# DanielaCourel/smoothed_particle_hydrodynamics

Hardware: AMD Instinct MI355X
Metric: Mparticle-steps/sec (whole node), dam-break (higher is better)
Workload: dtype f32

## Files before the change

smoothed_particle_hydrodynamics_amd/csrc/cell_build.h:

```cpp
#pragma once

#include "sph_device.h"

#define SCAN_THREADS 256
#ifndef RANK_UNROLL
#define RANK_UNROLL 4
#endif
#ifndef RANK_BIG
#define RANK_BIG 512
#endif
#define RANK_CHUNK 4096
#define RANK_BIG_BLOCKS 64
#define SCAN_ITEMS 16
#define SCAN_TILE (SCAN_THREADS * SCAN_ITEMS)

__device__ __forceinline__ void count_cell_runs(uint32_t c, bool live, int i,
                                                uint32_t* __restrict__ cell_count,
                                                uint32_t* __restrict__ slot, uint32_t trash)
{
   live = live && c != trash;
   const int lane = threadIdx.x & (SPH_WAVE - 1);
   const uint32_t prev = __shfl_up(c, 1);
   const bool head = (lane == 0) || (prev != c);
   const unsigned long long heads = __ballot(head);
   const unsigned long long below = heads & ((lane == 63) ? ~0ull : ((1ull << (lane + 1)) - 1ull));
   const int head_lane = 63 - __clzll(below);
   const unsigned long long above = (head_lane == 63) ? 0ull : (heads >> (head_lane + 1));
   const int run_len = above ? (__ffsll((long long)above)) : (SPH_WAVE - head_lane);
   uint32_t base = 0;
   if (live && head) base = atomicAdd(&cell_count[c], (uint32_t)run_len);
   base = __shfl(base, head_lane);
   if (live) slot[i] = base + (uint32_t)(lane - head_lane);
}

template <bool WRITE_VOX, bool CHECK_DEAD>
__global__ void __launch_bounds__(256)
k_hash_count(const float4* __restrict__ posm, const float4* __restrict__ velp,
             int32_t* __restrict__ meta, CellGrid g, SlabZone zone, uint32_t* __restrict__ key,
             uint32_t* __restrict__ slot, uint32_t* __restrict__ cell_count,
             int32_t* __restrict__ vox)
{
   const int i = blockIdx.x * blockDim.x + threadIdx.x;
   const bool live = i < meta[META_N_IN];
   uint32_t c = 0xffffffffu;
   if (live) {
      const float4 p = posm[i];
      int cx, cy, cz;
// ... 27 lines not shown
   count_cell_runs(c, live, i, cell_count, slot, (uint32_t)g.ncells);
}

__device__ __forceinline__ uint32_t wave_inclusive_scan(uint32_t v, int lane)
{
#pragma unroll
   for (int d = 1; d < SPH_WAVE; d <<= 1) {
      uint32_t t = __shfl_up(v, d);
      if (lane >= d) v += t;
   }
   return v;
}

__device__ __forceinline__ uint32_t block_exclusive_scan(uint32_t v, uint32_t* total)
{
   __shared__ uint32_t wave_sums[SCAN_THREADS / SPH_WAVE];
   const int lane = threadIdx.x & (SPH_WAVE - 1);
   const int w = threadIdx.x / SPH_WAVE;
   const uint32_t inc = wave_inclusive_scan(v, lane);
   if (lane == SPH_WAVE - 1) wave_sums[w] = inc;
   __syncthreads();
   uint32_t carry = 0, tot = 0;
#pragma unroll
   for (int k = 0; k < SCAN_THREADS / SPH_WAVE; k++) {
      const uint32_t s = wave_sums[k];
      if (k < w) carry += s;
      tot += s;
   }
   __syncthreads();
   *total = tot;
   return carry + inc - v;
}

__global__ void __launch_bounds__(SCAN_THREADS)
k_scan_reduce(const uint32_t* __restrict__ count, int ncells, uint32_t* __restrict__ part)
{
   const int base = blockIdx.x * SCAN_TILE + threadIdx.x * SCAN_ITEMS;
   uint32_t s = 0;
   if (base + SCAN_ITEMS <= ncells) {
      const uint4* p = reinterpret_cast<const uint4*>(count + base);
#pragma unroll
      for (int k = 0; k < SCAN_ITEMS / 4; k++) {
         const uint4 v = p[k];
         s += v.x + v.y + v.z + v.w;
      }
   } else {
      for (int k = 0; k < SCAN_ITEMS; k++)
         if (base + k < ncells) s += count[base + k];
   }
   uint32_t total;
   block_exclusive_scan(s, &total);
   if (threadIdx.x == 0) part[blockIdx.x] = total;
}

__global__ void __launch_bounds__(SCAN_THREADS)
k_scan_final(uint32_t* __restrict__ count, int ncells, const uint32_t* __restrict__ part,
             uint32_t* __restrict__ cell_start, uint32_t* __restrict__ big_cells, uint32_t limit,
             int32_t* __restrict__ meta)
{
   if (blockIdx.x == 0 && threadIdx.x == 0) big_cells[0] = 0u;
   const int base = blockIdx.x * SCAN_TILE + threadIdx.x * SCAN_ITEMS;
   uint32_t v[SCAN_ITEMS];
   uint32_t s = 0;
   const bool empty_tile = part[blockIdx.x] == 0u;
   if (empty_tile) {
#pragma unroll
      for (int k = 0; k < SCAN_ITEMS; k++) v[k] = 0u;
   } else if (base + SCAN_ITEMS <= ncells) {
      const uint4* p = reinterpret_cast<const uint4*>(count + base);
#pragma unroll
      for (int k = 0; k < SCAN_ITEMS / 4; k++) {
         const uint4 q = p[k];
         v[4 * k + 0] = q.x;
         v[4 * k + 1] = q.y;
         v[4 * k + 2] = q.z;
         v[4 * k + 3] = q.w;
      }
   } else {
#pragma unroll
      for (int k = 0; k < SCAN_ITEMS; k++) v[k] = (base + k < ncells) ? count[base + k] : 0u;
   }
#pragma unroll
   for (int k = 0; k < SCAN_ITEMS; k++) s += v[k];
   uint32_t before = 0;
   for (int t = threadIdx.x; t < (int)blockIdx.x; t += SCAN_THREADS) before += part[t];
   uint32_t carry;
   block_exclusive_scan(before, &carry);
   uint32_t total;
   uint32_t run = carry + block_exclusive_scan(s, &total);
   if (base + SCAN_ITEMS <= ncells) {
      uint4* o = reinterpret_cast<uint4*>(cell_start + base);
      uint4* z = reinterpret_cast<uint4*>(count + base);
#pragma unroll
      for (int k = 0; k < SCAN_ITEMS / 4; k++) {
         uint4 q;
         q.x = min(run, limit); run += v[4 * k + 0];
         q.y = min(run, limit); run += v[4 * k + 1];
         q.z = min(run, limit); run += v[4 * k + 2];
         q.w = min(run, limit); run += v[4 * k + 3];
         o[k] = q;
         if ((v[4 * k + 0] | v[4 * k + 1] | v[4 * k + 2] | v[4 * k + 3]) != 0u) z[k] = make_uint4(0, 0, 0, 0);
      }
   } else {
      for (int k = 0; k < SCAN_ITEMS; k++) {
         if (base + k < ncells) {
            cell_start[base + k] = min(run, limit);
            if (v[k] != 0u) count[base + k] = 0;
            run += v[k];
         }
      }
   }
   if (base <= ncells - 1 && ncells - 1 < base + SCAN_ITEMS) {
      cell_start[ncells] = min(run, limit);
      if (run > limit) atomicOr(&meta[META_ERRORS], 4);
   }
}

__global__ void __launch_bounds__(256)
k_scatter(const uint32_t* __restrict__ key, const uint32_t* __restrict__ slot,
          const uint32_t* __restrict__ cell_start, int32_t* __restrict__ meta,
          uint32_t* __restrict__ perm, int cells_per_plane, int ncells, int own_lo, int own_hi,
          int sum_lo, int sum_hi, int bnd_lo, int bnd_hi, int32_t* __restrict__ tile_stats,
          int32_t* __restrict__ clear_a, int32_t* __restrict__ clear_b,
          uint32_t* __restrict__ big_cells, uint32_t limit)
{
   const int i = blockIdx.x * blockDim.x + threadIdx.x;
   if (tile_stats && i < TSTAT_COUNT && i != TSTAT_BLOCKS) tile_stats[i] = 0;
   const int n_in = meta[META_N_IN];
   if (i < n_in) {
      const uint32_t c = key[i];
      if (c != (uint32_t)ncells) {
         const uint32_t first = cell_start[c], sl = slot[i];
         if (first + sl < limit) perm[first + sl] = (uint32_t)i;
         if (sl == 0u && cell_start[c + 1] - first > (uint32_t)RANK_BIG)
            big_cells[1u + atomicAdd(&big_cells[0], 1u)] = c;
      }
   }
   if (i == 0) {
      meta[META_N_LIVE] = (int)cell_start[ncells];
      meta[META_OWN_BEGIN] = (int)cell_start[own_lo * cells_per_plane];
      meta[META_OWN_END] = (int)cell_start[own_hi * cells_per_plane];
      meta[META_SUM_BEGIN] = (int)cell_start[sum_lo * cells_per_plane];
      meta[META_SUM_END] = (int)cell_start[sum_hi * cells_per_plane];
      meta[META_BND_LO_END] = (int)cell_start[bnd_lo * cells_per_plane];
      meta[META_BND_HI_BEGIN] = (int)cell_start[bnd_hi * cells_per_plane];
      if (clear_a) *clear_a = 0;
      if (clear_b) *clear_b = 0;
      if (tile_stats)
         tile_stats[TSTAT_BLOCKS] =
            (meta[META_SUM_END] - meta[META_SUM_BEGIN] + TILE_THREADS - 1) / TILE_THREADS;
   }
}

__global__ void __launch_bounds__(256)
k_rank_order(const uint32_t* __restrict__ perm, const uint32_t* __restrict__ key,
             const uint32_t* __restrict__ cell_start, const int32_t* __restrict__ meta,
             uint32_t* __restrict__ order)
{
   const int p = blockIdx.x * blockDim.x + threadIdx.x;
   if (p >= meta[META_N_IN]) return;
   const uint32_t i = perm[p];
   const uint32_t c = key[i];
   const uint32_t s = cell_start[c], e = cell_start[c + 1];
   if (e - s > (uint32_t)RANK_BIG) return;
   uint32_t rank = 0;
   for (uint32_t q0 = s; q0 < e; q0 += 8) {
      uint32_t other[8];
#pragma unroll
      for (int u = 0; u < 8; u++) other[u] = perm[q0 + u < e ? q0 + u : e - 1];
#pragma unroll
      for (int u = 0; u < 8; u++) rank += (q0 + u < e && other[u] < i) ? 1u : 0u;
   }
   order[s + rank] = i;
}

__device__ __forceinline__ void
rank_gather(int p, int block_p0, uint32_t* __restrict__ lds_id, const uint32_t* __restrict__ perm,
            const uint32_t* __restrict__ key, const uint32_t* __restrict__ cell_start,
            const int32_t* __restrict__ meta, int trash, const float4* __restrict__ posm_in,
            const float4* __restrict__ velp_in, float4* __restrict__ posm_out,
            float4* __restrict__ velp_out, uint32_t* __restrict__ remap = nullptr)
{
   const int n_in = (int)cell_start[trash];
   bool active = p < n_in;
   uint32_t i = 0, c = 0, s = 0, e = 0, id = 0;
   float4 v = make_float4(0.f, 0.f, 0.f, 0.f);
   if (active) {
      i = perm[p];
      c = key[i];
      v = velp_in[i];
      id = __float_as_uint(v.w);
   }
   lds_id[threadIdx.x] = id;
   if (active) {
      if (c == (uint32_t)trash) {
         active = false;
      } else {
         s = cell_start[c];
         e = cell_start[c + 1];
         if (e - s > (uint32_t)RANK_BIG) active = false;
      }
   }
   __syncthreads();
   if (!active) return;
   const uint32_t b0 = (uint32_t)block_p0;
   const uint32_t b1 = min(b0 + blockDim.x, (uint32_t)n_in);
   const uint32_t in_lo = max(s, b0), in_hi = min(e, b1);
   uint32_t rank = 0, same = 0;
   for (uint32_t q0 = in_lo; q0 < in_hi; q0 += 4) {
      uint32_t other[4];
#pragma unroll
      for (int u = 0; u < 4; u++) other[u] = lds_id[(q0 + u < in_hi ? q0 + u : in_hi - 1) - b0];
#pragma unroll
      for (int u = 0; u < 4; u++) {
         rank += (q0 + u < in_hi && other[u] < id) ? 1u : 0u;
         same += (q0 + u < in_hi && other[u] == id) ? 1u : 0u;
      }
   }
#pragma unroll
   for (int side = 0; side < 2; side++) {
      const uint32_t lo = side == 0 ? s : in_hi, hi = side == 0 ? in_lo : e;
      for (uint32_t q0 = lo; q0 < hi; q0 += RANK_UNROLL) {
         uint32_t other[RANK_UNROLL];
#pragma unroll
         for (int u = 0; u < RANK_UNROLL; u++) other[u] = perm[q0 + u < hi ? q0 + u : hi - 1];
#pragma unroll
         for (int u = 0; u < RANK_UNROLL; u++) other[u] = __float_as_uint(velp_in[other[u]].w);
#pragma unroll
         for (int u = 0; u < RANK_UNROLL; u++) {
            rank += (q0 + u < hi && other[u] < id) ? 1u : 0u;
            same += (q0 + u < hi && other[u] == id) ? 1u : 0u;
         }
      }
   }
   if (same > 1u) atomicOr(const_cast<int32_t*>(&meta[META_ERRORS]), 16);
   posm_out[s + rank] = posm_in[i];
   velp_out[s + rank] = v;
   if (remap) remap[i] = s + rank;
}

__global__ void __launch_bounds__(256)
k_rank_gather(const uint32_t* __restrict__ perm, const uint32_t* __restrict__ key,
              const uint32_t* __restrict__ cell_start, const int32_t* __restrict__ meta, int trash,
              const float4* __restrict__ posm_in, const float4* __restrict__ velp_in,
              float4* __restrict__ posm_out, float4* __restrict__ velp_out,
              uint32_t* __restrict__ remap)
{
   __shared__ uint32_t lds_id[256];
   rank_gather(blockIdx.x * blockDim.x + threadIdx.x, blockIdx.x * blockDim.x, lds_id, perm, key,
               cell_start, meta, trash, posm_in, velp_in, posm_out, velp_out, remap);
}

template <bool FULL>
__global__ void __launch_bounds__(256)
k_rank_big(const uint32_t* __restrict__ big_cells, const uint32_t* __restrict__ perm,
           const uint32_t* __restrict__ cell_start, const float4* __restrict__ posm_in,
           const float4* __restrict__ velp_in, float4* __restrict__ posm_out,
           float4* __restrict__ velp_out, uint32_t* __restrict__ order,
           uint32_t* __restrict__ scratch_key, uint32_t* __restrict__ scratch_src,
           uint32_t* __restrict__ remap)
{
   __shared__ uint32_t skey[RANK_CHUNK], ssrc[RANK_CHUNK];
   const int tid = threadIdx.x;
   const uint32_t nbig = big_cells[0];
   for (uint32_t b = blockIdx.x; b < nbig; b += gridDim.x) {
      const uint32_t c = big_cells[1u + b];
      const uint32_t s = cell_start[c], m = cell_start[c + 1] - s;
      const uint32_t nchunks = (m + RANK_CHUNK - 1) / RANK_CHUNK;
      for (uint32_t ch = 0; ch < nchunks; ch++) {
         const uint32_t base = ch * RANK_CHUNK;
         const uint32_t len = min((uint32_t)RANK_CHUNK, m - base);
         uint32_t padded = 256;
         while (padded < len) padded <<= 1;
         for (uint32_t t = tid; t < padded; t += 256) {
            uint32_t key = 0xffffffffu, src = 0u;
            if (t < len) {
               src = perm[s + base + t];
               key = FULL ? __float_as_uint(velp_in[src].w) : src;
            }
            skey[t] = key;
            ssrc[t] = src;
         }
         __syncthreads();
         for (uint32_t k2 = 2; k2 <= padded; k2 <<= 1) {
            for (uint32_t j = k2 >> 1; j > 0; j >>= 1) {
               for (uint32_t t = tid; t < padded; t += 256) {
                  const uint32_t partner = t ^ j;
                  if (partner > t) {
                     const bool up = (t & k2) == 0;
                     const uint32_t a = skey[t], bb = skey[partner];
                     if ((a > bb) == up) {
                        skey[t] = bb;
                        skey[partner] = a;
                        const uint32_t sa = ssrc[t];
                        ssrc[t] = ssrc[partner];
                        ssrc[partner] = sa;
                     }
                  }
               }
               __syncthreads();
            }
         }
         for (uint32_t t = tid; t < len; t += 256) {
            if (nchunks == 1) {
               const uint32_t src = ssrc[t];
               if (FULL) {
                  posm_out[s + t] = posm_in[src];
                  velp_out[s + t] = velp_in[src];
                  if (remap) remap[src] = s + t;
               } else {
                  order[s + t] = src;
               }
            } else {
               scratch_key[s + base + t] = skey[t];
               scratch_src[s + base + t] = ssrc[t];
            }
         }
         __syncthreads();
      }
      if (nchunks > 1) {
         for (uint32_t idx = tid; idx < m; idx += 256) {
            const uint32_t key = scratch_key[s + idx], mine = idx / RANK_CHUNK;
            uint32_t rank = idx % RANK_CHUNK;
            for (uint32_t ch = 0; ch < nchunks; ch++) {
               if (ch == mine) continue;
               const uint32_t* keys = scratch_key + s + ch * RANK_CHUNK;
               uint32_t lo = 0, hi = min((uint32_t)RANK_CHUNK, m - ch * RANK_CHUNK);
               while (lo < hi) {
                  const uint32_t mid = (lo + hi) >> 1;
                  if (keys[mid] < key) lo = mid + 1;
                  else hi = mid;
               }
               rank += lo;
            }
            const uint32_t src = scratch_src[s + idx];
            if (FULL) {
               posm_out[s + rank] = posm_in[src];
               velp_out[s + rank] = velp_in[src];
               if (remap) remap[src] = s + rank;
            } else {
               order[s + rank] = src;
            }
         }
         __syncthreads();
      }
   }
}

__global__ void __launch_bounds__(256)
k_permute_sums(const uint32_t* __restrict__ remap, const uint32_t* __restrict__ key,
               const int32_t* __restrict__ meta, uint32_t trash, const float* __restrict__ rho,
               const float4* __restrict__ acc, const int32_t* __restrict__ ncount,
               float* __restrict__ rho_out, float4* __restrict__ acc_out,
               int32_t* __restrict__ ncount_out)
{
   const int i = blockIdx.x * blockDim.x + threadIdx.x;
   if (i >= meta[META_N_IN] || key[i] == trash) return;
   const uint32_t j = remap[i];
   rho_out[j] = rho[i];
   acc_out[j] = acc[i];
   ncount_out[j] = ncount[i];
}
```

smoothed_particle_hydrodynamics_amd/csrc/context.h:

```cpp
#pragma once

#include <stdlib.h>
#include <string.h>

#include <memory>
#include <new>
#include <utility>

#include "cell_build.h"
#include "common_kernels.h"
#include "full_kernels.h"
#include "full_tiled.h"
#include "ref_kernels.h"
#include "sample_kernels.h"
#include "slab_kernels.h"
#include "slab_rccl.h"

namespace {

std::string g_create_error;

inline int div_up(int a, int b) { return (a + b - 1) / b; }

bool getenv_flag(const char* name)
// ... 83 lines not shown
   int growths = 0;

   ~SlabComm()
   {
      const RcclApi* api = comm ? rccl_api(nullptr) : nullptr;
      if (api) (void)api->CommDestroy(comm);
   }
};
#define SLAB_GROW_EVERY 16

struct sph_hip_context {
   sph_hip_params prm;
   int mode = 0;
   int device = 0;
   int capacity = 0;
   int n = 0;
   int n_owned = 0;
   DevBuf<int32_t> meta;
   int plane_lo = 0, plane_hi = 0, halo = 0;
   hipStream_t stream = nullptr;
   Stream own_stream;
   Event ev[EV_RING][7];
   long long ev_steps = 0;
   std::string err;

   CellGrid grid;

   DevBuf<float4> posm[2];
   DevBuf<float4> velp[2];
   int cur = 0;

   DevBuf<uint32_t> key;
   DevBuf<uint32_t> slot;
   DevBuf<uint32_t> perm;
   DevBuf<uint32_t> order;
   DevBuf<uint32_t> cell_count;
   DevBuf<uint32_t> cell_start;
   DevBuf<uint32_t> scan_part;
   DevBuf<uint32_t> big_cells;
   int scan_tiles = 0;

   DevBuf<float> rho;
   DevBuf<float4> velB;
   DevBuf<float> auxc;
   DevBuf<float4> acc;
   DevBuf<int32_t> ncount;
   DevBuf<TileDesc> tile_desc;
   DevBuf<uint32_t> nlist;
   DevBuf<uint32_t> nlist_overflow;
   int fast = 0;
   struct {
      int valid = 0;
      int fast = 0;
      float rho0 = 0.0f, stiffness = 0.0f, kernel3 = 0.0f;
   } terms;
   int uniform_mass = 0;
   int use_tiled = 1;
   int prehashed = 0;
   int no_prehash = 0, no_fused_integrate = 0, no_fused_slab = 0;
   Stream chunk_stream;
   Event ev_chunk_fork, ev_chunk_join;
   int chunked_giveups = -1;
   int slab_fused = 0;
   void* slab_msgs[2] = {nullptr, nullptr};
   int slab_msg_capacity = 0;
   int had_exchange = 0;
   int may_hold_dead = 0;
// ... 238 lines not shown
```

smoothed_particle_hydrodynamics_amd/csrc/full_tiled.h:

```cpp
#pragma once

#include "launch_policy.h"
#include "common_kernels.h"
#include "full_kernels.h"
#include "slab_kernels.h"

#if defined(SPH_ABLATE) && !defined(SPH_DIAGNOSTIC_BUILD)
#error "SPH_ABLATE is for diagnostic builds only: add -DSPH_DIAGNOSTIC_BUILD (tools/build_variant.sh does)"
#endif

#ifdef SPH_TRIPCOUNT
#ifndef SPH_DIAGNOSTIC_BUILD
#error "SPH_TRIPCOUNT is for diagnostic builds only: add -DSPH_DIAGNOSTIC_BUILD"
#endif
enum {
   TRIP_D_WAVES = 0, TRIP_D_CHUNKS_W, TRIP_D_TEST8_W, TRIP_D_TEST8_L, TRIP_D_SLOTS_L, TRIP_D_POPS_W,
   TRIP_D_POPS_L, TRIP_D_POPLOOPS_W, TRIP_D_SUMTRIPS_W, TRIP_D_SUMSLOTS_W, TRIP_D_LISTED_L, TRIP_D_LANES_L,
   TRIP_A_WAVES = 16, TRIP_A_PTRIPS_W, TRIP_A_CNT_L, TRIP_A_VTRIPS_W, TRIP_A_NV_L, TRIP_A_LANES_L,
   TRIP_COUNT = 32
};
__device__ unsigned long long g_trip[TRIP_COUNT];
struct TripCounters {
   unsigned int v[16];
   __device__ TripCounters() { for (int i = 0; i < 16; i++) v[i] = 0; }
// ... 127 lines not shown
      return d.D[k];
   }
};

typedef float __attribute__((ext_vector_type(2))) f32x2;
typedef float __attribute__((ext_vector_type(4))) f32x4;

__device__ __forceinline__ f32x4 lds_read4(const float* base, int i)
{
   return *reinterpret_cast<const f32x4*>(__builtin_assume_aligned(base + i, 16));
}

static_assert(DENSITY_UNROLL == LIST_BLOCK_ENTRIES && ACCEL_UNROLL == LIST_BLOCK_ENTRIES, "a trip of the list-driven loops is one block of the lists");
static_assert(TILE_CAP_MAX + TILE_PAD <= (1 << ListEntry<false>::TBITS) &&
                 TILE_CAP_MAX_WIDE + TILE_PAD <= (1 << ListEntry<true>::TBITS),
              "tile index must fit the list entry");

struct TileDesc {
   int D[9];
   int B[9];
   int total;
   int pad;
};

struct TileLds {
   float* x;
   float* y;
   float* z;
};

extern __shared__ __attribute__((aligned(16))) float tile_lds_dynamic[];

__device__ __forceinline__ void
tile_desc(int tile, int ntiles, const uint32_t* __restrict__ perm, const uint32_t* __restrict__ key,
          const uint32_t* __restrict__ cell_start, const int32_t* __restrict__ meta, CellGrid g,
          TileDesc* __restrict__ desc, const TileCaps& caps, int32_t* __restrict__ stats,
          uint32_t* __restrict__ giveup_density, uint32_t* __restrict__ giveup_accel)
{
   const int begin = meta[META_SUM_BEGIN], end = meta[META_SUM_END];
   const int p0 = begin + tile * TILE_THREADS;
   int most = -1;
   if (tile < ntiles && p0 < end) {
      const int plast = min(p0 + TILE_THREADS - 1, end - 1);
      const int c_first = (int)key[perm[p0]];
      const int c_last = (int)key[perm[plast]];
      TileDesc d;
      int G[9], len[9];
#pragma unroll
      for (int k = 0; k < 9; k++) {
         const int off = ((k / 3 - 1) * g.ny + (k % 3 - 1)) * g.nx;
         int lo = c_first + off - 1, hi = c_last + off + 1;
         lo = lo < 0 ? 0 : lo;
         hi = hi > g.ncells - 1 ? g.ncells - 1 : hi;
         G[k] = 0;
         len[k] = 0;
         if (hi >= lo) {
            G[k] = (int)cell_start[lo];
            len[k] = (int)cell_start[hi + 1] - G[k];
         }
      }
      int run = 0, chain_end = -1, chain_d = 0;
#pragma unroll
      for (int k = 0; k < 9; k++) {
         d.B[k] = run;
         if (len[k] == 0) {
            d.D[k] = run - G[k];
         } else if (G[k] <= chain_end) {
            const int seg_end = G[k] + len[k];
            d.D[k] = chain_d;
            if (seg_end > chain_end) {
               run += seg_end - chain_end;
               chain_end = seg_end;
            }
         } else {
            d.D[k] = chain_d = run - G[k];
            run += len[k];
            chain_end = G[k] + len[k];
         }
      }
      d.total = run;
      d.pad = 0;
      desc[tile] = d;
      most = run;
   }
   const bool lead = (threadIdx.x & (SPH_WAVE - 1)) == 0;
#pragma unroll
   for (int c = 0; c < TILE_CANDS; c++) {
      const int over = __popcll(__ballot(c < caps.n_cand && most > caps.cand[c]));
      if (lead && over) atomicAdd(&stats[TSTAT_OVER + c], over);
   }
   int wave_most = most;
#pragma unroll
   for (int o = SPH_WAVE / 2; o > 0; o >>= 1) wave_most = max(wave_most, __shfl_xor(wave_most, o));
   if (lead && wave_most > stats[TSTAT_MAX]) atomicMax(&stats[TSTAT_MAX], wave_most);
   if (most > caps.cap_density) giveup_density[atomicAdd(&stats[TSTAT_GIVEUP_DENSITY], 1)] = (uint32_t)tile;
   if (most > caps.cap_density || most > caps.cap_accel)
      giveup_accel[atomicAdd(&stats[TSTAT_GIVEUP_ACCEL], 1)] = (uint32_t)tile;
}

__global__ void __launch_bounds__(256)
k_rank_gather_tile_desc(int desc_blocks, int ntiles, const uint32_t* __restrict__ perm,
                        const uint32_t* __restrict__ key, const uint32_t* __restrict__ cell_start,
                        const int32_t* __restrict__ meta, CellGrid g,
                        const float4* __restrict__ posm_in, const float4* __restrict__ velp_in,
                        float4* __restrict__ posm_out, float4* __restrict__ velp_out,
                        TileDesc* __restrict__ desc, TileCaps caps, int32_t* __restrict__ stats,
                        uint32_t* __restrict__ giveup_density, uint32_t* __restrict__ giveup_accel,
                        uint32_t* __restrict__ remap)
{
   if ((int)blockIdx.x < desc_blocks) {
      tile_desc(blockIdx.x * blockDim.x + threadIdx.x, ntiles, perm, key, cell_start, meta, g, desc,
                caps, stats, giveup_density, giveup_accel);
      return;
   }
   __shared__ uint32_t lds_id[256];
   rank_gather((blockIdx.x - desc_blocks) * blockDim.x + threadIdx.x,
               (blockIdx.x - desc_blocks) * blockDim.x, lds_id, perm, key, cell_start, meta,
               g.ncells, posm_in, velp_in, posm_out, velp_out, remap);
}

__device__ __forceinline__ void tile_desc_load(const TileDesc* __restrict__ desc, int wg, TileDesc& sd)
{
   const int tid = threadIdx.x;
   if (tid < (int)(sizeof(TileDesc) / sizeof(int)))
      reinterpret_cast<int*>(&sd)[tid] = reinterpret_cast<const int*>(&desc[wg])[tid];
   __syncthreads();
}

__device__ __forceinline__ int xcd_workgroup(int block, int nblocks)
{
   const int q = nblocks / 8, r = nblocks % 8, x = block % 8;
   return (x < r ? x * (q + 1) : r * (q + 1) + (x - r) * q) + block / 8;
}

__device__ __forceinline__ void tile_load(const float4* __restrict__ posm, const TileDesc& sd,
                                          const TileLds& L)
{
   const int tid = threadIdx.x;
   const int total = sd.total;
   int B[9], D[9];
#pragma unroll
   for (int k = 0; k < 9; k++) {
      B[k] = sd.B[k];
      D[k] = sd.D[k];
   }
#if defined(SPH_ABLATE) && (SPH_ABLATE == 3 || SPH_ABLATE == 5)
   for (int base = 0; base < 0; base += TILE_BATCH * TILE_THREADS) {
#else
   for (int base = 0; base < total; base += TILE_BATCH * TILE_THREADS) {
#endif
      float4 buf[TILE_BATCH];
// ... 1070 lines not shown
```

smoothed_particle_hydrodynamics_amd/csrc/launch.h:

```cpp
#pragma once

#include <math.h>

#include <type_traits>

#include "context.h"

namespace {

template <class F>
void bind_flags(F&& f) { f(); }
template <class F, class... Rest>
void bind_flags(F&& f, bool flag, Rest... rest)
{
   if (flag) bind_flags([&](auto... later) { f(std::true_type{}, later...); }, rest...);
   else bind_flags([&](auto... later) { f(std::false_type{}, later...); }, rest...);
}

PairConsts pair_consts(const sph_hip_params& p, bool fast)
{
   PairConsts k;
   k.h2 = p.h2;
   static const float screen = getenv("SPH_HIP_TEST_SCREEN") ? (float)atof(getenv("SPH_HIP_TEST_SCREEN"))
                                                             : TEST_SCREEN_FACTOR;
// ... 172 lines not shown
   const SlabZone zone = slab_zone(ctx);
   if (ctx->prehashed == 2) {
      ctx->prehashed = 0;
      hipLaunchKernelGGL(k_hash_tail, dim3(SLAB_PACK_BLOCKS), dim3(256), 0, st, ctx->posm[cur], ctx->meta, g,
                         ctx->key, ctx->slot, ctx->cell_count);
   } else if (ctx->prehashed) {
      ctx->prehashed = 0;
   } else {
      const bool ref = ctx->mode == SPH_HIP_MODE_REF;
      bind_flags([&](auto R, auto D) {
         if constexpr (!(R.value && D.value))
            hipLaunchKernelGGL((k_hash_count<R.value, D.value>), dim3(blocks), dim3(256), 0, st, ctx->posm[cur],
                               ctx->velp[cur], ctx->meta, g, zone, ctx->key, ctx->slot, ctx->cell_count,
                               R.value ? ctx->vox.get() : nullptr);
      }, ref, !ref && ctx->may_hold_dead != 0);
   }
   ctx->early_exchange = 0;
   ctx->may_hold_dead = 0;
   const int tiles = ctx->scan_tiles;
   const int ncells_scan = g.ncells + 1;
   hipLaunchKernelGGL(k_scan_reduce, dim3(tiles), dim3(SCAN_THREADS), 0, st, ctx->cell_count,
                      ncells_scan, ctx->scan_part);
   hipLaunchKernelGGL(k_scan_final, dim3(tiles), dim3(SCAN_THREADS), 0, st, ctx->cell_count,
                      ncells_scan, ctx->scan_part, ctx->cell_start, ctx->big_cells, (uint32_t)ctx->capacity,
                      ctx->meta);
   const PlaneRanges r = plane_ranges(ctx->plane_lo, ctx->plane_hi, g.z0, g.nz, ctx->halo, zone.have_left,
                                      zone.have_right);
   hipLaunchKernelGGL(k_scatter, dim3(blocks), dim3(256), 0, st, ctx->key, ctx->slot,
                      ctx->cell_start, ctx->meta, ctx->perm, g.nx * g.ny, g.ncells, r.own_lo, r.own_hi,
                      r.sum_lo, r.sum_hi, r.bnd_lo, r.bnd_hi, ctx->tile_stats, (int32_t*)clear_left,
                      (int32_t*)clear_right, ctx->big_cells, (uint32_t)ctx->capacity);
   uint32_t* scratch_key = reinterpret_cast<uint32_t*>(ctx->stage.get());
   uint32_t* scratch_src = scratch_key + ctx->capacity;
   uint32_t* remap = (keep_sums && ctx->mode == SPH_HIP_MODE_FULL && !ctx->had_exchange) ? ctx->slot : nullptr;
   if (ctx->mode == SPH_HIP_MODE_REF) {
      hipLaunchKernelGGL(k_rank_order, dim3(blocks), dim3(256), 0, st, ctx->perm, ctx->key,
                         ctx->cell_start, ctx->meta, ctx->order);
      hipLaunchKernelGGL(k_rank_big<false>, dim3(RANK_BIG_BLOCKS), dim3(256), 0, st, ctx->big_cells,
                         ctx->perm, ctx->cell_start, (const float4*)nullptr, (const float4*)nullptr,
                         (float4*)nullptr, (float4*)nullptr, ctx->order, scratch_key, scratch_src,
                         (uint32_t*)nullptr);
   } else {
      const int nxt = cur ^ 1;
      if (ctx->use_tiled) {
         static_assert(sizeof(TileDesc) == 20 * sizeof(int), "TileDesc is 20 ints");
         pick_tile_caps(ctx);
         const int ntiles = div_up(n, TILE_THREADS), desc_blocks = div_up(ntiles, 256);
         hipLaunchKernelGGL(k_rank_gather_tile_desc, dim3(desc_blocks + blocks), dim3(256), 0, st,
                            desc_blocks, ntiles, ctx->perm, ctx->key, ctx->cell_start, ctx->meta,
                            g, ctx->posm[cur], ctx->velp[cur], ctx->posm[nxt], ctx->velp[nxt],
                            ctx->tile_desc, ctx->caps, ctx->tile_stats, ctx->giveup_density,
                            ctx->giveup_accel, remap);
      } else {
         hipLaunchKernelGGL(k_rank_gather, dim3(blocks), dim3(256), 0, st, ctx->perm, ctx->key,
                            ctx->cell_start, ctx->meta, g.ncells, ctx->posm[cur], ctx->velp[cur],
                            ctx->posm[nxt], ctx->velp[nxt], remap);
      }
      hipLaunchKernelGGL(k_rank_big<true>, dim3(RANK_BIG_BLOCKS), dim3(256), 0, st, ctx->big_cells,
                         ctx->perm, ctx->cell_start, ctx->posm[cur], ctx->velp[cur], ctx->posm[nxt],
                         ctx->velp[nxt], (uint32_t*)nullptr, scratch_key, scratch_src, remap);
      if (remap) {
         ctx->terms.valid = 0;
         float4* acc_t = reinterpret_cast<float4*>(ctx->stage.get() + ((2 * (size_t)ctx->capacity + 3) & ~(size_t)3));
         float* rho_t = reinterpret_cast<float*>(acc_t + (size_t)ctx->capacity);
         int32_t* cnt_t = reinterpret_cast<int32_t*>(rho_t + (size_t)ctx->capacity);
         hipLaunchKernelGGL(k_permute_sums, dim3(blocks), dim3(256), 0, st, remap, ctx->key, ctx->meta,
                            (uint32_t)g.ncells, ctx->rho, ctx->acc, ctx->ncount, rho_t, acc_t, cnt_t);
         SPH_TRY(hipMemcpyAsync(ctx->rho, rho_t, sizeof(float) * n, hipMemcpyDeviceToDevice, st));
         SPH_TRY(hipMemcpyAsync(ctx->acc, acc_t, sizeof(float4) * n, hipMemcpyDeviceToDevice, st));
         SPH_TRY(hipMemcpyAsync(ctx->ncount, cnt_t, sizeof(int32_t) * n, hipMemcpyDeviceToDevice, st));
      }
      ctx->cur = nxt;
   }
   SPH_TRY(hipGetLastError());
   return SPH_HIP_OK;
}

int launch_find_neighbors(sph_hip_context* ctx)
{
   if (ctx->mode != SPH_HIP_MODE_REF || ctx->n == 0) return SPH_HIP_OK;
   const sph_hip_params& p = ctx->prm;
   hipLaunchKernelGGL(k_ref_find_neighbors, dim3(div_up(ctx->n, 256)), dim3(256), 0, ctx->stream,
                      ctx->posm[0], ctx->vox, ctx->cell_start, ctx->order, ctx->n, p.cells_x,
                      p.cells_y, p.cells_z, p.h, p.htimes2, p.h2, p.sim_scale, p.examine_count,
                      ctx->nb, ctx->nd, ctx->ncount);
   SPH_TRY(hipGetLastError());
   return SPH_HIP_OK;
}

struct SlabFused {
   void* left;
   void* right;
   int capacity;
// ... 291 lines not shown
```

Measured before the change: 4796.

## Pack cell id into perm, fuse big-cell ranking into gather kernel, restructure scan

The permutation array now stores the particle index and its cell id as a pair, so the rank, gather and tile-descriptor code no longer chase key[perm[p]]. The big-cell sort runs as extra leading blocks of the gather kernel (using a smaller LDS chunk) instead of a separate launch. Rank-gather finds cell bounds within its block from LDS run heads, which avoids most cell_start loads. The cell scan processes twice as many cells per tile with a wave-strided, coalesced uint4 layout. In exchange, perm traffic doubles, and the big-cell blocks now share LDS sizing and scheduling with the normal gather blocks.

```diff
diff --git a/smoothed_particle_hydrodynamics_amd/csrc/cell_build.h b/smoothed_particle_hydrodynamics_amd/csrc/cell_build.h
--- a/smoothed_particle_hydrodynamics_amd/csrc/cell_build.h
+++ b/smoothed_particle_hydrodynamics_amd/csrc/cell_build.h
@@ -11,8 +11,12 @@
 #endif
 #define RANK_CHUNK 4096
 #define RANK_BIG_BLOCKS 64
-#define SCAN_ITEMS 16
+#ifndef SCAN_ITEMS
+#define SCAN_ITEMS 32
+#endif
 #define SCAN_TILE (SCAN_THREADS * SCAN_ITEMS)
+#define SCAN_WAVE_CELLS (SCAN_TILE / (SCAN_THREADS / SPH_WAVE))
+#define SCAN_ROUNDS (SCAN_WAVE_CELLS / (4 * SPH_WAVE))
 
 __device__ __forceinline__ void count_cell_runs(uint32_t c, bool live, int i,
                                                 uint32_t* __restrict__ cell_count,
@@ -106,22 +110,32 @@
    return carry + inc - v;
 }
 
+__device__ __forceinline__ int scan_cell0(int tile)
+{
+   return tile * SCAN_TILE + (threadIdx.x / SPH_WAVE) * SCAN_WAVE_CELLS + 4 * (threadIdx.x & (SPH_WAVE - 1));
+}
+
+__device__ __forceinline__ uint4 scan_load4(const uint32_t* __restrict__ count, int c0, int ncells)
+{
+   if (c0 + 4 <= ncells) return *reinterpret_cast<const uint4*>(count + c0);
+   uint4 q;
+   q.x = c0 + 0 < ncells ? count[c0 + 0] : 0u;
+   q.y = c0 + 1 < ncells ? count[c0 + 1] : 0u;
+   q.z = c0 + 2 < ncells ? count[c0 + 2] : 0u;
+   q.w = c0 + 3 < ncells ? count[c0 + 3] : 0u;
+   return q;
+}
+
 __global__ void __launch_bounds__(SCAN_THREADS)
 k_scan_reduce(const uint32_t* __restrict__ count, int ncells, uint32_t* __restrict__ part)
 {
-   const int base = blockIdx.x * SCAN_TILE + threadIdx.x * SCAN_ITEMS;
+   const int cell0 = scan_cell0(blockIdx.x);
+   uint4 q[SCAN_ROUNDS];
+#pragma unroll
+   for (int r = 0; r < SCAN_ROUNDS; r++) q[r] = scan_load4(count, cell0 + r * 4 * SPH_WAVE, ncells);
    uint32_t s = 0;
-   if (base + SCAN_ITEMS <= ncells) {
-      const uint4* p = reinterpret_cast<const uint4*>(count + base);
-#pragma unroll
-      for (int k = 0; k < SCAN_ITEMS / 4; k++) {
-         const uint4 v = p[k];
-         s += v.x + v.y + v.z + v.w;
-      }
-   } else {
-      for (int k = 0; k < SCAN_ITEMS; k++)
-         if (base + k < ncells) s += count[base + k];
-   }
+#pragma unroll
+   for (int r = 0; r < SCAN_ROUNDS; r++) s += q[r].x + q[r].y + q[r].z + q[r].w;
    uint32_t total;
    block_exclusive_scan(s, &total);
    if (threadIdx.x == 0) part[blockIdx.x] = total;
@@ -133,67 +147,61 @@
              int32_t* __restrict__ meta)
 {
    if (blockIdx.x == 0 && threadIdx.x == 0) big_cells[0] = 0u;
-   const int base = blockIdx.x * SCAN_TILE + threadIdx.x * SCAN_ITEMS;
-   uint32_t v[SCAN_ITEMS];
-   uint32_t s = 0;
+   const int lane = threadIdx.x & (SPH_WAVE - 1);
+   const int cell0 = scan_cell0(blockIdx.x);
    const bool empty_tile = part[blockIdx.x] == 0u;
-   if (empty_tile) {
-#pragma unroll
-      for (int k = 0; k < SCAN_ITEMS; k++) v[k] = 0u;
-   } else if (base + SCAN_ITEMS <= ncells) {
-      const uint4* p = reinterpret_cast<const uint4*>(count + base);
-#pragma unroll
-      for (int k = 0; k < SCAN_ITEMS / 4; k++) {
-         const uint4 q = p[k];
-         v[4 * k + 0] = q.x;
-         v[4 * k + 1] = q.y;
-         v[4 * k + 2] = q.z;
-         v[4 * k + 3] = q.w;
-      }
-   } else {
-#pragma unroll
-      for (int k = 0; k < SCAN_ITEMS; k++) v[k] = (base + k < ncells) ? count[base + k] : 0u;
-   }
-#pragma unroll
-   for (int k = 0; k < SCAN_ITEMS; k++) s += v[k];
+   uint4 q[SCAN_ROUNDS];
+#pragma unroll
+   for (int r = 0; r < SCAN_ROUNDS; r++)
+      q[r] = empty_tile ? make_uint4(0, 0, 0, 0) : scan_load4(count, cell0 + r * 4 * SPH_WAVE, ncells);
    uint32_t before = 0;
    for (int t = threadIdx.x; t < (int)blockIdx.x; t += SCAN_THREADS) before += part[t];
    uint32_t carry;
    block_exclusive_scan(before, &carry);
+   uint32_t pre[SCAN_ROUNDS];
+   uint32_t wave_run = 0;
+#pragma unroll
+   for (int r = 0; r < SCAN_ROUNDS; r++) {
+      const uint32_t sum = q[r].x + q[r].y + q[r].z + q[r].w;
+      const uint32_t inc = wave_inclusive_scan(sum, lane);
+      pre[r] = wave_run + inc - sum;
+      wave_run += __shfl(inc, SPH_WAVE - 1);
+   }
    uint32_t total;
-   uint32_t run = carry + block_exclusive_scan(s, &total);
-   if (base + SCAN_ITEMS <= ncells) {
-      uint4* o = reinterpret_cast<uint4*>(cell_start + base);
-      uint4* z = reinterpret_cast<uint4*>(count + base);
-#pragma unroll
-      for (int k = 0; k < SCAN_ITEMS / 4; k++) {
-         uint4 q;
-         q.x = min(run, limit); run += v[4 * k + 0];
-         q.y = min(run, limit); run += v[4 * k + 1];
-         q.z = min(run, limit); run += v[4 * k + 2];
-         q.w = min(run, limit); run += v[4 * k + 3];
-         o[k] = q;
-         if ((v[4 * k + 0] | v[4 * k + 1] | v[4 * k + 2] | v[4 * k + 3]) != 0u) z[k] = make_uint4(0, 0, 0, 0);
-      }
-   } else {
-      for (int k = 0; k < SCAN_ITEMS; k++) {
-         if (base + k < ncells) {
-            cell_start[base + k] = min(run, limit);
-            if (v[k] != 0u) count[base + k] = 0;
-            run += v[k];
-         }
-      }
-   }
-   if (base <= ncells - 1 && ncells - 1 < base + SCAN_ITEMS) {
-      cell_start[ncells] = min(run, limit);
-      if (run > limit) atomicOr(&meta[META_ERRORS], 4);
+   const uint32_t run = carry + __shfl(block_exclusive_scan(lane == 0 ? wave_run : 0u, &total), 0);
+#pragma unroll
+   for (int r = 0; r < SCAN_ROUNDS; r++) {
+      const int c0 = cell0 + r * 4 * SPH_WAVE;
+      const uint32_t v[4] = {q[r].x, q[r].y, q[r].z, q[r].w};
+      uint32_t at = run + pre[r];
+      if (c0 + 4 <= ncells) {
+         uint4 o;
+         o.x = min(at, limit); at += v[0];
+         o.y = min(at, limit); at += v[1];
+         o.z = min(at, limit); at += v[2];
+         o.w = min(at, limit); at += v[3];
+         *reinterpret_cast<uint4*>(cell_start + c0) = o;
+         if ((v[0] | v[1] | v[2] | v[3]) != 0u) *reinterpret_cast<uint4*>(count + c0) = make_uint4(0, 0, 0, 0);
+      } else {
+         for (int k = 0; k < 4; k++) {
+            if (c0 + k < ncells) {
+               cell_start[c0 + k] = min(at, limit);
+               if (v[k] != 0u) count[c0 + k] = 0;
+               at += v[k];
+            }
+         }
+      }
+      if (c0 <= ncells - 1 && ncells - 1 < c0 + 4) {
+         cell_start[ncells] = min(at, limit);
+         if (at > limit) atomicOr(&meta[META_ERRORS], 4);
+      }
    }
 }
 
 __global__ void __launch_bounds__(256)
 k_scatter(const uint32_t* __restrict__ key, const uint32_t* __restrict__ slot,
           const uint32_t* __restrict__ cell_start, int32_t* __restrict__ meta,
-          uint32_t* __restrict__ perm, int cells_per_plane, int ncells, int own_lo, int own_hi,
+          uint2* __restrict__ perm, int cells_per_plane, int ncells, int own_lo, int own_hi,
           int sum_lo, int sum_hi, int bnd_lo, int bnd_hi, int32_t* __restrict__ tile_stats,
           int32_t* __restrict__ clear_a, int32_t* __restrict__ clear_b,
           uint32_t* __restrict__ big_cells, uint32_t limit)
@@ -205,7 +213,7 @@
       const uint32_t c = key[i];
       if (c != (uint32_t)ncells) {
          const uint32_t first = cell_start[c], sl = slot[i];
-         if (first + sl < limit) perm[first + sl] = (uint32_t)i;
+         if (first + sl < limit) perm[first + sl] = make_uint2((uint32_t)i, c);
          if (sl == 0u && cell_start[c + 1] - first > (uint32_t)RANK_BIG)
             big_cells[1u + atomicAdd(&big_cells[0], 1u)] = c;
       }
@@ -227,59 +235,76 @@
 }
 
 __global__ void __launch_bounds__(256)
-k_rank_order(const uint32_t* __restrict__ perm, const uint32_t* __restrict__ key,
-             const uint32_t* __restrict__ cell_start, const int32_t* __restrict__ meta,
+k_rank_order(const uint2* __restrict__ perm, const uint32_t* __restrict__ cell_start, int trash,
              uint32_t* __restrict__ order)
 {
    const int p = blockIdx.x * blockDim.x + threadIdx.x;
-   if (p >= meta[META_N_IN]) return;
-   const uint32_t i = perm[p];
-   const uint32_t c = key[i];
+   if (p >= (int)cell_start[trash]) return;
+   const uint2 pc = perm[p];
+   const uint32_t i = pc.x, c = pc.y;
    const uint32_t s = cell_start[c], e = cell_start[c + 1];
    if (e - s > (uint32_t)RANK_BIG) return;
    uint32_t rank = 0;
    for (uint32_t q0 = s; q0 < e; q0 += 8) {
       uint32_t other[8];
 #pragma unroll
-      for (int u = 0; u < 8; u++) other[u] = perm[q0 + u < e ? q0 + u : e - 1];
+      for (int u = 0; u < 8; u++) other[u] = perm[q0 + u < e ? q0 + u : e - 1].x;
 #pragma unroll
       for (int u = 0; u < 8; u++) rank += (q0 + u < e && other[u] < i) ? 1u : 0u;
    }
    order[s + rank] = i;
 }
 
+#define RANK_GATHER_WAVES (256 / SPH_WAVE)
+#define RANK_GATHER_LDS (2 * 256 + 2 * RANK_GATHER_WAVES)
 __device__ __forceinline__ void
-rank_gather(int p, int block_p0, uint32_t* __restrict__ lds_id, const uint32_t* __restrict__ perm,
-            const uint32_t* __restrict__ key, const uint32_t* __restrict__ cell_start,
-            const int32_t* __restrict__ meta, int trash, const float4* __restrict__ posm_in,
-            const float4* __restrict__ velp_in, float4* __restrict__ posm_out,
-            float4* __restrict__ velp_out, uint32_t* __restrict__ remap = nullptr)
-{
+rank_gather(int p, int block_p0, uint32_t* __restrict__ lds, const uint2* __restrict__ perm,
+            const uint32_t* __restrict__ cell_start, const int32_t* __restrict__ meta, int trash,
+            const float4* __restrict__ posm_in, const float4* __restrict__ velp_in,
+            float4* __restrict__ posm_out, float4* __restrict__ velp_out,
+            uint32_t* __restrict__ remap = nullptr)
+{
+   uint32_t* lds_c = lds;
+   uint32_t* lds_id = lds + 256;
+   int* wave_first = reinterpret_cast<int*>(lds + 512);
+   int* wave_last = wave_first + RANK_GATHER_WAVES;
+   const int tid = threadIdx.x, lane = tid & (SPH_WAVE - 1), w = tid / SPH_WAVE;
    const int n_in = (int)cell_start[trash];
    bool active = p < n_in;
-   uint32_t i = 0, c = 0, s = 0, e = 0, id = 0;
-   float4 v = make_float4(0.f, 0.f, 0.f, 0.f);
+   uint32_t i = 0, c = 0xffffffffu, id = 0;
+   float4 v = make_float4(0.f, 0.f, 0.f, 0.f), x = v;
    if (active) {
-      i = perm[p];
-      c = key[i];
+      const uint2 pc = perm[p];
+      i = pc.x;
+      c = pc.y;
       v = velp_in[i];
+      x = posm_in[i];
       id = __float_as_uint(v.w);
    }
-   lds_id[threadIdx.x] = id;
-   if (active) {
-      if (c == (uint32_t)trash) {
-         active = false;
-      } else {
-         s = cell_start[c];
-         e = cell_start[c + 1];
-         if (e - s > (uint32_t)RANK_BIG) active = false;
-      }
-   }
+   lds_c[tid] = c;
+   lds_id[tid] = id;
    __syncthreads();
-   if (!active) return;
+   const unsigned long long heads = __ballot(active && (tid == 0 || lds_c[tid - 1] != c));
+   if (lane == 0) {
+      wave_first[w] = heads ? w * SPH_WAVE + __ffsll((long long)heads) - 1 : 256;
+      wave_last[w] = heads ? w * SPH_WAVE + 63 - __clzll(heads) : -1;
+   }
+   __syncthreads();
+   if (!active || c == (uint32_t)trash) return;
+   const int nb = min(256, n_in - block_p0);
+   const unsigned long long below = heads & ((lane == 63) ? ~0ull : ((1ull << (lane + 1)) - 1ull));
+   int lo_l = below ? w * SPH_WAVE + 63 - __clzll(below) : 0;
+   if (!below)
+      for (int k = 0; k < w; k++) lo_l = max(lo_l, wave_last[k]);
+   const unsigned long long above = (lane == 63) ? 0ull : (heads >> (lane + 1));
+   int hi_l = above ? tid + __ffsll((long long)above) : nb;
+   if (!above)
+      for (int k = w + 1; k < RANK_GATHER_WAVES; k++) hi_l = min(hi_l, wave_first[k]);
    const uint32_t b0 = (uint32_t)block_p0;
-   const uint32_t b1 = min(b0 + blockDim.x, (uint32_t)n_in);
-   const uint32_t in_lo = max(s, b0), in_hi = min(e, b1);
+   const uint32_t in_lo = b0 + (uint32_t)lo_l, in_hi = b0 + (uint32_t)hi_l;
+   const uint32_t s = lo_l == 0 ? cell_start[c] : in_lo;
+   const uint32_t e = hi_l == nb ? cell_start[c + 1] : in_hi;
+   if (e - s > (uint32_t)RANK_BIG) return;
    uint32_t rank = 0, same = 0;
    for (uint32_t q0 = in_lo; q0 < in_hi; q0 += 4) {
       uint32_t other[4];
@@ -297,7 +322,7 @@
       for (uint32_t q0 = lo; q0 < hi; q0 += RANK_UNROLL) {
          uint32_t other[RANK_UNROLL];
 #pragma unroll
-         for (int u = 0; u < RANK_UNROLL; u++) other[u] = perm[q0 + u < hi ? q0 + u : hi - 1];
+         for (int u = 0; u < RANK_UNROLL; u++) other[u] = perm[q0 + u < hi ? q0 + u : hi - 1].x;
 #pragma unroll
          for (int u = 0; u < RANK_UNROLL; u++) other[u] = __float_as_uint(velp_in[other[u]].w);
 #pragma unroll
@@ -308,48 +333,36 @@
       }
    }
    if (same > 1u) atomicOr(const_cast<int32_t*>(&meta[META_ERRORS]), 16);
-   posm_out[s + rank] = posm_in[i];
+   posm_out[s + rank] = x;
    velp_out[s + rank] = v;
    if (remap) remap[i] = s + rank;
 }
 
-__global__ void __launch_bounds__(256)
-k_rank_gather(const uint32_t* __restrict__ perm, const uint32_t* __restrict__ key,
-              const uint32_t* __restrict__ cell_start, const int32_t* __restrict__ meta, int trash,
-              const float4* __restrict__ posm_in, const float4* __restrict__ velp_in,
-              float4* __restrict__ posm_out, float4* __restrict__ velp_out,
-              uint32_t* __restrict__ remap)
-{
-   __shared__ uint32_t lds_id[256];
-   rank_gather(blockIdx.x * blockDim.x + threadIdx.x, blockIdx.x * blockDim.x, lds_id, perm, key,
-               cell_start, meta, trash, posm_in, velp_in, posm_out, velp_out, remap);
-}
-
-template <bool FULL>
-__global__ void __launch_bounds__(256)
-k_rank_big(const uint32_t* __restrict__ big_cells, const uint32_t* __restrict__ perm,
-           const uint32_t* __restrict__ cell_start, const float4* __restrict__ posm_in,
-           const float4* __restrict__ velp_in, float4* __restrict__ posm_out,
-           float4* __restrict__ velp_out, uint32_t* __restrict__ order,
-           uint32_t* __restrict__ scratch_key, uint32_t* __restrict__ scratch_src,
-           uint32_t* __restrict__ remap)
-{
-   __shared__ uint32_t skey[RANK_CHUNK], ssrc[RANK_CHUNK];
+template <bool FULL, int CHUNK>
+__device__ void
+rank_big_cells(int block, int nblocks, uint32_t* __restrict__ skey, uint32_t* __restrict__ ssrc,
+               const uint32_t* __restrict__ big_cells, const uint2* __restrict__ perm,
+               const uint32_t* __restrict__ cell_start, const float4* __restrict__ posm_in,
+               const float4* __restrict__ velp_in, float4* __restrict__ posm_out,
+               float4* __restrict__ velp_out, uint32_t* __restrict__ order,
+               uint32_t* __restrict__ scratch_key, uint32_t* __restrict__ scratch_src,
+               uint32_t* __restrict__ remap)
+{
    const int tid = threadIdx.x;
    const uint32_t nbig = big_cells[0];
-   for (uint32_t b = blockIdx.x; b < nbig; b += gridDim.x) {
+   for (uint32_t b = block; b < nbig; b += nblocks) {
       const uint32_t c = big_cells[1u + b];
       const uint32_t s = cell_start[c], m = cell_start[c + 1] - s;
-      const uint32_t nchunks = (m + RANK_CHUNK - 1) / RANK_CHUNK;
+      const uint32_t nchunks = (m + CHUNK - 1) / CHUNK;
       for (uint32_t ch = 0; ch < nchunks; ch++) {
-         const uint32_t base = ch * RANK_CHUNK;
-         const uint32_t len = min((uint32_t)RANK_CHUNK, m - base);
+         const uint32_t base = ch * CHUNK;
+         const uint32_t len = min((uint32_t)CHUNK, m - base);
          uint32_t padded = 256;
          while (padded < len) padded <<= 1;
          for (uint32_t t = tid; t < padded; t += 256) {
             uint32_t key = 0xffffffffu, src = 0u;
             if (t < len) {
-               src = perm[s + base + t];
+               src = perm[s + base + t].x;
                key = FULL ? __float_as_uint(velp_in[src].w) : src;
             }
             skey[t] = key;
@@ -394,12 +407,12 @@
       }
       if (nchunks > 1) {
          for (uint32_t idx = tid; idx < m; idx += 256) {
-            const uint32_t key = scratch_key[s + idx], mine = idx / RANK_CHUNK;
-            uint32_t rank = idx % RANK_CHUNK;
+            const uint32_t key = scratch_key[s + idx], mine = idx / CHUNK;
+            uint32_t rank = idx % CHUNK;
             for (uint32_t ch = 0; ch < nchunks; ch++) {
                if (ch == mine) continue;
-               const uint32_t* keys = scratch_key + s + ch * RANK_CHUNK;
-               uint32_t lo = 0, hi = min((uint32_t)RANK_CHUNK, m - ch * RANK_CHUNK);
+               const uint32_t* keys = scratch_key + s + ch * CHUNK;
+               uint32_t lo = 0, hi = min((uint32_t)CHUNK, m - ch * CHUNK);
                while (lo < hi) {
                   const uint32_t mid = (lo + hi) >> 1;
                   if (keys[mid] < key) lo = mid + 1;
@@ -422,6 +435,56 @@
 }
 
 __global__ void __launch_bounds__(256)
+k_rank_big(const uint32_t* __restrict__ big_cells, const uint2* __restrict__ perm,
+           const uint32_t* __restrict__ cell_start, uint32_t* __restrict__ order,
+           uint32_t* __restrict__ scratch_key, uint32_t* __restrict__ scratch_src)
+{
+   __shared__ uint32_t skey[RANK_CHUNK], ssrc[RANK_CHUNK];
+   rank_big_cells<false, RANK_CHUNK>(blockIdx.x, gridDim.x, skey, ssrc, big_cells, perm, cell_start,
+                                     nullptr, nullptr, nullptr, nullptr, order, scratch_key, scratch_src,
+                                     nullptr);
+}
+
+#define RANK_CHUNK_GATHER 2048
+#define RANK_GATHER_SHARED (2 * RANK_CHUNK_GATHER)
+static_assert(RANK_GATHER_SHARED >= RANK_GATHER_LDS, "the big-cell sort's LDS holds the gather's");
+
+struct BigCellWork {
+   const uint32_t* big_cells;
+   uint32_t* scratch_key;
+   uint32_t* scratch_src;
+};
+
+__device__ __forceinline__ void
+gather_big_cells(int block, uint32_t* __restrict__ lds, const BigCellWork& big,
+                 const uint2* __restrict__ perm, const uint32_t* __restrict__ cell_start,
+                 const float4* __restrict__ posm_in, const float4* __restrict__ velp_in,
+                 float4* __restrict__ posm_out, float4* __restrict__ velp_out,
+                 uint32_t* __restrict__ remap)
+{
+   rank_big_cells<true, RANK_CHUNK_GATHER>(block, RANK_BIG_BLOCKS, lds, lds + RANK_CHUNK_GATHER,
+                                           big.big_cells, perm, cell_start, posm_in, velp_in, posm_out,
+                                           velp_out, nullptr, big.scratch_key, big.scratch_src, remap);
+}
+
+__global__ void __launch_bounds__(256)
+k_rank_gather(BigCellWork big, const uint2* __restrict__ perm,
+              const uint32_t* __restrict__ cell_start, const int32_t* __restrict__ meta, int trash,
+              const float4* __restrict__ posm_in, const float4* __restrict__ velp_in,
+              float4* __restrict__ posm_out, float4* __restrict__ velp_out,
+              uint32_t* __restrict__ remap)
+{
+   __shared__ uint32_t lds[RANK_GATHER_SHARED];
+   if ((int)blockIdx.x < RANK_BIG_BLOCKS) {
+      gather_big_cells(blockIdx.x, lds, big, perm, cell_start, posm_in, velp_in, posm_out, velp_out, remap);
+      return;
+   }
+   const int b = blockIdx.x - RANK_BIG_BLOCKS;
+   rank_gather(b * blockDim.x + threadIdx.x, b * blockDim.x, lds, perm, cell_start, meta, trash, posm_in,
+               velp_in, posm_out, velp_out, remap);
+}
+
+__global__ void __launch_bounds__(256)
 k_permute_sums(const uint32_t* __restrict__ remap, const uint32_t* __restrict__ key,
                const int32_t* __restrict__ meta, uint32_t trash, const float* __restrict__ rho,
                const float4* __restrict__ acc, const int32_t* __restrict__ ncount,
diff --git a/smoothed_particle_hydrodynamics_amd/csrc/context.h b/smoothed_particle_hydrodynamics_amd/csrc/context.h
--- a/smoothed_particle_hydrodynamics_amd/csrc/context.h
+++ b/smoothed_particle_hydrodynamics_amd/csrc/context.h
@@ -139,7 +139,7 @@
 
    DevBuf<uint32_t> key;
    DevBuf<uint32_t> slot;
-   DevBuf<uint32_t> perm;
+   DevBuf<uint2> perm;
    DevBuf<uint32_t> order;
    DevBuf<uint32_t> cell_count;
    DevBuf<uint32_t> cell_start;
diff --git a/smoothed_particle_hydrodynamics_amd/csrc/full_tiled.h b/smoothed_particle_hydrodynamics_amd/csrc/full_tiled.h
--- a/smoothed_particle_hydrodynamics_amd/csrc/full_tiled.h
+++ b/smoothed_particle_hydrodynamics_amd/csrc/full_tiled.h
@@ -183,7 +183,7 @@
 extern __shared__ __attribute__((aligned(16))) float tile_lds_dynamic[];
 
 __device__ __forceinline__ void
-tile_desc(int tile, int ntiles, const uint32_t* __restrict__ perm, const uint32_t* __restrict__ key,
+tile_desc(int tile, int ntiles, const uint2* __restrict__ perm,
           const uint32_t* __restrict__ cell_start, const int32_t* __restrict__ meta, CellGrid g,
           TileDesc* __restrict__ desc, const TileCaps& caps, int32_t* __restrict__ stats,
           uint32_t* __restrict__ giveup_density, uint32_t* __restrict__ giveup_accel)
@@ -193,8 +193,8 @@
    int most = -1;
    if (tile < ntiles && p0 < end) {
       const int plast = min(p0 + TILE_THREADS - 1, end - 1);
-      const int c_first = (int)key[perm[p0]];
-      const int c_last = (int)key[perm[plast]];
+      const int c_first = (int)perm[p0].y;
+      const int c_last = (int)perm[plast].y;
       TileDesc d;
       int G[9], len[9];
 #pragma unroll
@@ -250,8 +250,8 @@
 }
 
 __global__ void __launch_bounds__(256)
-k_rank_gather_tile_desc(int desc_blocks, int ntiles, const uint32_t* __restrict__ perm,
-                        const uint32_t* __restrict__ key, const uint32_t* __restrict__ cell_start,
+k_rank_gather_tile_desc(BigCellWork big, int desc_blocks, int ntiles, const uint2* __restrict__ perm,
+                        const uint32_t* __restrict__ cell_start,
                         const int32_t* __restrict__ meta, CellGrid g,
                         const float4* __restrict__ posm_in, const float4* __restrict__ velp_in,
                         float4* __restrict__ posm_out, float4* __restrict__ velp_out,
@@ -259,15 +259,21 @@
                         uint32_t* __restrict__ giveup_density, uint32_t* __restrict__ giveup_accel,
                         uint32_t* __restrict__ remap)
 {
-   if ((int)blockIdx.x < desc_blocks) {
-      tile_desc(blockIdx.x * blockDim.x + threadIdx.x, ntiles, perm, key, cell_start, meta, g, desc,
-                caps, stats, giveup_density, giveup_accel);
+   __shared__ uint32_t lds[RANK_GATHER_SHARED];
+   int b = blockIdx.x;
+   if (b < RANK_BIG_BLOCKS) {
+      gather_big_cells(b, lds, big, perm, cell_start, posm_in, velp_in, posm_out, velp_out, remap);
       return;
    }
-   __shared__ uint32_t lds_id[256];
-   rank_gather((blockIdx.x - desc_blocks) * blockDim.x + threadIdx.x,
-               (blockIdx.x - desc_blocks) * blockDim.x, lds_id, perm, key, cell_start, meta,
-               g.ncells, posm_in, velp_in, posm_out, velp_out, remap);
+   b -= RANK_BIG_BLOCKS;
+   if (b < desc_blocks) {
+      tile_desc(b * blockDim.x + threadIdx.x, ntiles, perm, cell_start, meta, g, desc, caps, stats,
+                giveup_density, giveup_accel);
+      return;
+   }
+   b -= desc_blocks;
+   rank_gather(b * blockDim.x + threadIdx.x, b * blockDim.x, lds, perm, cell_start, meta, g.ncells,
+               posm_in, velp_in, posm_out, velp_out, remap);
 }
 
 __device__ __forceinline__ void tile_desc_load(const TileDesc* __restrict__ desc, int wg, TileDesc& sd)
diff --git a/smoothed_particle_hydrodynamics_amd/csrc/launch.h b/smoothed_particle_hydrodynamics_amd/csrc/launch.h
--- a/smoothed_particle_hydrodynamics_amd/csrc/launch.h
+++ b/smoothed_particle_hydrodynamics_amd/csrc/launch.h
@@ -228,33 +228,29 @@
                       (int32_t*)clear_right, ctx->big_cells, (uint32_t)ctx->capacity);
    uint32_t* scratch_key = reinterpret_cast<uint32_t*>(ctx->stage.get());
    uint32_t* scratch_src = scratch_key + ctx->capacity;
+   const BigCellWork big{ctx->big_cells, scratch_key, scratch_src};
    uint32_t* remap = (keep_sums && ctx->mode == SPH_HIP_MODE_FULL && !ctx->had_exchange) ? ctx->slot : nullptr;
    if (ctx->mode == SPH_HIP_MODE_REF) {
-      hipLaunchKernelGGL(k_rank_order, dim3(blocks), dim3(256), 0, st, ctx->perm, ctx->key,
-                         ctx->cell_start, ctx->meta, ctx->order);
-      hipLaunchKernelGGL(k_rank_big<false>, dim3(RANK_BIG_BLOCKS), dim3(256), 0, st, ctx->big_cells,
-                         ctx->perm, ctx->cell_start, (const float4*)nullptr, (const float4*)nullptr,
-                         (float4*)nullptr, (float4*)nullptr, ctx->order, scratch_key, scratch_src,
-                         (uint32_t*)nullptr);
+      hipLaunchKernelGGL(k_rank_order, dim3(blocks), dim3(256), 0, st, ctx->perm, ctx->cell_start,
+                         g.ncells, ctx->order);
+      hipLaunchKernelGGL(k_rank_big, dim3(RANK_BIG_BLOCKS), dim3(256), 0, st, ctx->big_cells, ctx->perm,
+                         ctx->cell_start, ctx->order, scratch_key, scratch_src);
    } else {
       const int nxt = cur ^ 1;
       if (ctx->use_tiled) {
          static_assert(sizeof(TileDesc) == 20 * sizeof(int), "TileDesc is 20 ints");
          pick_tile_caps(ctx);
          const int ntiles = div_up(n, TILE_THREADS), desc_blocks = div_up(ntiles, 256);
-         hipLaunchKernelGGL(k_rank_gather_tile_desc, dim3(desc_blocks + blocks), dim3(256), 0, st,
-                            desc_blocks, ntiles, ctx->perm, ctx->key, ctx->cell_start, ctx->meta,
+         hipLaunchKernelGGL(k_rank_gather_tile_desc, dim3(RANK_BIG_BLOCKS + desc_blocks + blocks), dim3(256),
+                            0, st, big, desc_blocks, ntiles, ctx->perm, ctx->cell_start, ctx->meta,
                             g, ctx->posm[cur], ctx->velp[cur], ctx->posm[nxt], ctx->velp[nxt],
                             ctx->tile_desc, ctx->caps, ctx->tile_stats, ctx->giveup_density,
                             ctx->giveup_accel, remap);
       } else {
-         hipLaunchKernelGGL(k_rank_gather, dim3(blocks), dim3(256), 0, st, ctx->perm, ctx->key,
+         hipLaunchKernelGGL(k_rank_gather, dim3(RANK_BIG_BLOCKS + blocks), dim3(256), 0, st, big, ctx->perm,
                             ctx->cell_start, ctx->meta, g.ncells, ctx->posm[cur], ctx->velp[cur],
                             ctx->posm[nxt], ctx->velp[nxt], remap);
       }
-      hipLaunchKernelGGL(k_rank_big<true>, dim3(RANK_BIG_BLOCKS), dim3(256), 0, st, ctx->big_cells,
-                         ctx->perm, ctx->cell_start, ctx->posm[cur], ctx->velp[cur], ctx->posm[nxt],
-                         ctx->velp[nxt], (uint32_t*)nullptr, scratch_key, scratch_src, remap);
       if (remap) {
          ctx->terms.valid = 0;
          float4* acc_t = reinterpret_cast<float4*>(ctx->stage.get() + ((2 * (size_t)ctx->capacity + 3) & ~(size_t)3));
```

After: 4817 (median of 6 runs). About the same (+0.4%).
